# ACEfanatic02/par_raytracer

Hardware: AMD Instinct MI355X
Metric: Mrays/s at 1920x1080x8spp, 1M-tri OBJ (higher is better)
Workload: dtype f32; 1 GPU; C4: synthetic 1,002,528-triangle terrain OBJ (1,024 groups), 1920x1080, 8 spp, bounce_depth 2; seed=1234, triangles=1002528, width=1920, height=1080, spp=8, bounce_depth=2, rays_per_frame=77049910, parallelism=pixel rows sharded in 8-row blocks over 1 GPU(s), pipeline=pool, frames_in_flight=1

## Files before the change

par_raytracer_amd/csrc/dev_trace4.h:

```cpp
#pragma once

#include "dev_trace_common.h"

namespace prt {

struct TravRay {
    f3 o, d;
    float ix, iy, iz;
    float pnx, pny, pnz;
    HitRec best;
    int node, sp, kind;
};


enum { TRAV_SENTINEL = (int)0x80000000, TRAV_FLAG_NEAR = 1, TRAV_FLAG_OVERFLOW = 2, TRAV_SENTINEL_LAST = (int)0x80000003 };
PRT_D bool trav_done(int node) { return node <= TRAV_SENTINEL_LAST; }
PRT_D bool trav_flagged(int node) { return node <= TRAV_SENTINEL_LAST && node != TRAV_SENTINEL; }

typedef int StackEntry;
enum { STACK_ENTRY_INTS = 1, BVH_NODE_BYTES = 64, STACK_LDS_CAP_DEFAULT = 24 };

template <int BLOCK>
struct LdsStack {
    int * col;
    unsigned int cap;
    PRT_D void attach(int * lds, unsigned int tid) { col = lds + tid; }
    PRT_D int * frame_col() const { return col; }
    PRT_D bool push(int sp, int v) const {
        if ((unsigned int)sp < cap) { col[sp * BLOCK] = v; return true; }
        return false;
    }
    PRT_D int pop(int sp) const { return col[sp * BLOCK]; }
    PRT_D void flag(int bit) const { col[0] |= bit; }
};

template <int BLOCK>
struct LdsSpillStack {
    int * col;
    unsigned int cap;
    PRT_D void attach(int * lds, unsigned int tid) { col = lds + tid; }
    PRT_D int * frame_col() const { return col; }
    PRT_D void set_spill(int * base, unsigned int lanes) { spill = base; spill_stride = lanes; }
    int * spill;
    unsigned int spill_stride;
    PRT_D size_t spill_index(int sp) const {
        return (size_t)((unsigned int)sp - cap) * spill_stride + (blockIdx.x * (unsigned int)BLOCK + threadIdx.x);
    }
    PRT_D bool push(int sp, int v) const {
        if ((unsigned int)sp < cap) col[sp * BLOCK] = v;
        else spill[spill_index(sp)] = v;
        return true;
    }
    PRT_D int pop(int sp) const {
        if ((unsigned int)sp < cap) return col[sp * BLOCK];
        return spill[spill_index(sp)];
    }
    PRT_D void flag(int bit) const { col[0] |= bit; }
};

struct GlobalStack {
    int * col;
    size_t stride;
    PRT_D void attach(int * base, size_t lane, size_t lanes) { col = base + lane; stride = lanes; }
    PRT_D bool push(int sp, int v) const { col[(size_t)sp * stride] = v; return true; }
    PRT_D int pop(int sp) const { return col[(size_t)sp * stride]; }
    PRT_D void flag(int bit) const { col[0] |= bit; }
};

PRT_D void trav_idle(TravRay & r) { r.node = TRAV_SENTINEL; r.sp = 0; r.kind = 0; }
PRT_D bool trav_walking(const TravRay & r) { return r.node >= 0; }
PRT_D bool trav_done(const TravRay & r) { return trav_done(r.node); }

template <class STK> PRT_D int trav_end_flags(const TravRay & r, const STK &) { return trav_done(r.node) ? (r.node & 3) : 0; }
template <class STK> PRT_D bool trav_wants_resolve(const TravRay & r, const STK & stk) { return r.kind == TRACE_CLOSEST && (trav_end_flags(r, stk) & TRAV_FLAG_NEAR) != 0 && r.best.tri >= 0; }
template <class STK> PRT_D bool trav_needs_slow_path(const TravRay & r, const STK & stk) { return (trav_end_flags(r, stk) & TRAV_FLAG_OVERFLOW) != 0 || trav_wants_resolve(r, stk); }

template <class STK>
PRT_D void trav_pop(TravRay & r, const STK & stk) {
    r.sp--;
    r.node = stk.pop(r.sp);
}
template <class STK>
PRT_D void trav_push(TravRay & r, const STK & stk, int link) {
    if (stk.push(r.sp, link)) r.sp++;
    else stk.flag(TRAV_FLAG_OVERFLOW);
}

template <class STK>
PRT_D void trav_init(TravRay & r, f3 o, f3 d, int kind, float pad, const STK & stk) {
    r.o = o;
    r.d = d;
    const float tiny = 1e-30f;
    float dx = fabsf(d.x) < tiny ? (d.x < 0.0f ? -tiny : tiny) : d.x;
    float dy = fabsf(d.y) < tiny ? (d.y < 0.0f ? -tiny : tiny) : d.y;
    float dz = fabsf(d.z) < tiny ? (d.z < 0.0f ? -tiny : tiny) : d.z;
    r.ix = 1.0f / dx; r.iy = 1.0f / dy; r.iz = 1.0f / dz;
    r.pnx = (dx < 0.0f ? o.x - pad : o.x + pad) * r.ix;
    r.pny = (dy < 0.0f ? o.y - pad : o.y + pad) * r.iy;
    r.pnz = (dz < 0.0f ? o.z - pad : o.z + pad) * r.iz;
    r.best.t = 3.402823466e+38f;
    r.best.v = r.best.w = 0.0f;
    r.best.tri = -1;
    r.kind = kind;
    stk.push(0, TRAV_SENTINEL);
    r.sp = 1;
    r.node = 0;
}

PRT_D void cswap(float & ka, float & kb, int & la, int & lb) {
    const bool sw = kb < ka;
    const float k0 = sw ? kb : ka, k1 = sw ? ka : kb;
    const int l0 = sw ? lb : la, l1 = sw ? la : lb;
    ka = k0; kb = k1; la = l0; lb = l1;
}

template <class STK, bool COUNT>
PRT_D void trav_node_step(const DevScene & sc, TravRay & r, const STK & stk, TraceStats & st, float pad) {
    const uint4 * np = reinterpret_cast<const uint4 *>(reinterpret_cast<const char *>(sc.nodes) + ((unsigned int)r.node << 6));
    const uint4 w0 = np[0], w1 = np[1], w2 = np[2], w3 = np[3];
    if (COUNT) { st.nodes++; if (first_active_lane()) st.wnodes++; if ((unsigned int)r.sp > st.max_sp) st.max_sp = (unsigned int)r.sp; }
    const float kx = __uint_as_float(w0.w) * r.ix;
    const float ky = __uint_as_float(w3.z) * r.iy;
    const float kz = __uint_as_float(w3.w) * r.iz;
    const float ox = __uint_as_float(w0.x), oy = __uint_as_float(w0.y), oz = __uint_as_float(w0.z);
    const float pad2 = pad + pad;
    const float cnx = __builtin_fmaf(ox, r.ix, -r.pnx), cfx = __builtin_fmaf(pad2, fabsf(r.ix), cnx);
    const float cny = __builtin_fmaf(oy, r.iy, -r.pny), cfy = __builtin_fmaf(pad2, fabsf(r.iy), cny);
    const float cnz = __builtin_fmaf(oz, r.iz, -r.pnz), cfz = __builtin_fmaf(pad2, fabsf(r.iz), cnz);
    const bool sx = r.ix < 0.0f, sy = r.iy < 0.0f, sz = r.iz < 0.0f;
    const unsigned int qnx = sx ? w1.w : w1.x, qfx = sx ? w1.x : w1.w;
    const unsigned int qny = sy ? w2.x : w1.y, qfy = sy ? w1.y : w2.x;
    const unsigned int qnz = sz ? w2.y : w1.z, qfz = sz ? w1.z : w2.y;
    float key[4];
    int link[4] = { (int)w2.z, (int)w2.w, (int)w3.x, (int)w3.y };
    const float inf = __uint_as_float(0x7F800000u);
#pragma unroll
    for (int k = 0; k < 4; ++k) {
        const float nx = __builtin_fmaf((float)((qnx >> (8 * k)) & 0xFFu), kx, cnx);
        const float fx = __builtin_fmaf((float)((qfx >> (8 * k)) & 0xFFu), kx, cfx);
        const float ny = __builtin_fmaf((float)((qny >> (8 * k)) & 0xFFu), ky, cny);
        const float fy = __builtin_fmaf((float)((qfy >> (8 * k)) & 0xFFu), ky, cfy);
        const float nz = __builtin_fmaf((float)((qnz >> (8 * k)) & 0xFFu), kz, cnz);
        const float fz = __builtin_fmaf((float)((qfz >> (8 * k)) & 0xFFu), kz, cfz);
        const float tmin = fmaxf(fmaxf(fmaxf(nx, ny), nz), 0.0f);
        const float tmax = fminf(fminf(fminf(fx, fy), fz), r.best.t);
        key[k] = tmin <= tmax ? tmin : inf;
    }
    cswap(key[0], key[1], link[0], link[1]);
    cswap(key[2], key[3], link[2], link[3]);
    cswap(key[0], key[2], link[0], link[2]);
    cswap(key[1], key[3], link[1], link[3]);
    cswap(key[1], key[2], link[1], link[2]);
    if (key[0] < inf) {
        if (COUNT && first_active_lane()) st.wdescend++;
        if (COUNT) {
            const unsigned long long p3 = __ballot(key[3] < inf), p2 = __ballot(key[2] < inf), p1 = __ballot(key[1] < inf);
            if (first_active_lane()) st.wpush += (unsigned int)(p3 != 0ull) + (unsigned int)(p2 != 0ull) + (unsigned int)(p1 != 0ull);
        }
        if (key[3] < inf) trav_push(r, stk, link[3]);
        if (key[2] < inf) trav_push(r, stk, link[2]);
        if (key[1] < inf) trav_push(r, stk, link[1]);
        r.node = link[0];
    } else {
        if (COUNT && r.best.tri >= 0) st.culled++;
        if (COUNT && first_active_lane()) st.wpop++;
        trav_pop(r, stk);
    }
}

template <class STK, bool COUNT>
PRT_D bool trav_leaf(const DevScene & sc, TravRay & r, const STK & stk, TraceStats & st) {
    const f3 qp = r.o - (r.o + r.d);
    const unsigned int leaf = (unsigned int)~r.node;
    const unsigned int first = leaf >> 2, count = (leaf & 3u) + 1u;
    if (COUNT) { if (first_active_lane()) st.wleaves++; }
    int next_node = stk.pop(r.sp - 1);
    bool flagged = false;
    for (unsigned int i = 0; i < count; ++i) {
        const unsigned int ti = first + i;
        const float4 * tp = reinterpret_cast<const float4 *>(reinterpret_cast<const char *>(sc.tris) + ti * 48u);
        const float4 r0 = tp[0], r1 = tp[1], r2 = tp[2];
#if defined(__HIP_DEVICE_COMPILE__)
        asm volatile("" :: "v"(r0.x), "v"(r0.y), "v"(r0.z));
#endif
        if (COUNT) { st.tris++; if (first_active_lane()) st.wtris++; }
        float t, v, w;
        bool near;
        const bool hit = tri_test(r.o, r.d, qp, mk3(r0.x, r0.y, r0.z), mk3(r0.w, r1.x, r1.y), mk3(r1.z, r1.w, r2.x),
                                  mk3(r2.y, r2.z, r2.w), r.best.t, t, v, w, near);
        if (near) {
            stk.flag(TRAV_FLAG_NEAR);
            flagged = true;
        }
        if (hit) {
            r.best.t = t;
            r.best.v = v;
            r.best.w = w;
            r.best.tri = (int)ti;
            if (r.kind & TRACE_ANY) return true;
        }
    }
    if (flagged && r.sp == 1) next_node |= TRAV_FLAG_NEAR;
    r.sp--;
    r.node = next_node;
    return false;
}

template <class STK, bool COUNT>
PRT_D HitRec resolve_near_ties(const DevScene & sc, f3 o, f3 d, float pad, float min_t, const STK & stk, TraceStats & st) {
    TravRay r;
    HitRec result;
    result.t = 3.402823466e+38f; result.v = result.w = 0.0f; result.tri = -1;
    const f3 qp = o - (o + d);
    float bound = min_t * PRT_TIE_NEAR;
    for (unsigned int widen = 0; ; ++widen) {
        const bool last = widen >= sc.tie_widen_max;
        const float moat = bound * 1.00000095367431640625f;
        bool occupied = false;
        float best = 3.402823466e+38f;
        result.tri = -1;
        unsigned int next_rank = 0;
        RefSphereWalk walk;
        walk.reset();
        for (;;) {
            unsigned int c_rank = 0xFFFFFFFFu;
            int c_tri = -1;
            trav_init(r, o, d, TRACE_CLOSEST, pad, stk);
            r.best.t = moat;
            for (;;) {
                while (r.node >= 0) trav_node_step<STK, COUNT>(sc, r, stk, st, pad);
                if (trav_done(r.node)) break;
                const unsigned int leaf = (unsigned int)~r.node;
                const unsigned int first = leaf >> 2, count = (leaf & 3u) + 1u;
                for (unsigned int i = 0; i < count; ++i) {
                    const unsigned int ti = first + i;
                    const float4 * tp = sc.tris + 3 * (size_t)ti;
                    const float4 r0 = tp[0], r1 = tp[1], r2 = tp[2];
                    float t, dd, v, w;
                    if (!tri_geom(o, qp, mk3(r0.x, r0.y, r0.z), mk3(r0.w, r1.x, r1.y), mk3(r1.z, r1.w, r2.x), mk3(r2.y, r2.z, r2.w), t, dd, v, w)) continue;
                    const float th = t * (1.0f / dd);
                    if (th > bound) { if (th <= moat) occupied = true; continue; }
                    const unsigned int rk = sc.tri_rank[ti];
                    if (rk >= next_rank && rk < c_rank) { c_rank = rk; c_tri = (int)ti; }
                }
                trav_pop(r, stk);
            }
            if (c_tri < 0 || (occupied && !last)) break;
            const float4 * tp = sc.tris + 3 * (size_t)c_tri;
            const float4 r0 = tp[0], r1 = tp[1], r2 = tp[2];
            float t, v, w;
            if (walk.offers(sc, o, d, c_rank, best) &&
                tri_test_ref(o, qp, mk3(r0.x, r0.y, r0.z), mk3(r0.w, r1.x, r1.y), mk3(r1.z, r1.w, r2.x), mk3(r2.y, r2.z, r2.w), best, t, v, w)) {
                best = t;
                result.t = t; result.v = v; result.w = w; result.tri = c_tri;
            }
            next_rank = c_rank + 1u;
        }
        if (!occupied) break;
        if (last) {
            if (sc.near_tie_unresolved) atomicAdd(sc.near_tie_unresolved, 1ull);
            break;
        }
        bound = moat * PRT_TIE_NEAR;
    }
    return result;
}

template <class STK, bool COUNT>
PRT_D HitRec trace_ray(const DevScene & sc, f3 o, f3 d, int kind, float pad, const STK & stk, TraceStats & st) {
    TravRay r;
    trav_init(r, o, d, kind, pad, stk);
    for (;;) {
        while (r.node >= 0) trav_node_step<STK, COUNT>(sc, r, stk, st, pad);
        if (trav_done(r.node)) break;
        if (trav_leaf<STK, COUNT>(sc, r, stk, st)) return r.best;
    }
    if (kind == TRACE_CLOSEST && (r.node & TRAV_FLAG_NEAR) && r.best.tri >= 0) return resolve_near_ties<STK, COUNT>(sc, o, d, pad, r.best.t, stk, st);
    return r.best;
}

}
```

par_raytracer_amd/csrc/dev_trace8.h:

```cpp
#pragma once

#include "dev_trace_common.h"

namespace prt {

typedef int2 StackEntry;
enum { STACK_ENTRY_INTS = 2, BVH_NODE_BYTES = 80, STACK_LDS_CAP_DEFAULT = 13 };

struct TravRay {
    f3 o, d;
    float ix, iy, iz;
    float pnx, pny, pnz;
    HitRec best;
    int node;
    unsigned int tbase;
    unsigned int tbits;
    int sp, kind;
};

enum { TRAV_SENTINEL = (int)0x80000000, TRAV_FLAG_NEAR = 1, TRAV_FLAG_OVERFLOW = 2, TRAV_SENTINEL_LAST = (int)0x80000003 };

template <int BLOCK>
struct LdsStack {
    int * col;
    unsigned int cap;
    PRT_D void attach(int * lds, unsigned int tid) { col = lds + tid; }
    PRT_D int * frame_col() const { return col; }
    PRT_D bool put(int sp, int2 v) const {
        if ((unsigned int)sp < cap) { col[(2 * sp) * BLOCK] = v.x; col[(2 * sp + 1) * BLOCK] = v.y; return true; }
        return false;
    }
    PRT_D int2 get(int sp) const { return make_int2(col[(2 * sp) * BLOCK], col[(2 * sp + 1) * BLOCK]); }
    PRT_D void flag(int bit) const { col[0] |= bit; }
    PRT_D int marker() const { return col[0]; }
};

template <int BLOCK>
struct LdsSpillStack {
    int * col;
    unsigned int cap;
    int2 * spill;
    unsigned int spill_stride;
    PRT_D void attach(int * lds, unsigned int tid) { col = lds + tid; }
    PRT_D int * frame_col() const { return col; }
    PRT_D void set_spill(int * base, unsigned int lanes) { spill = reinterpret_cast<int2 *>(base); spill_stride = lanes; }
    PRT_D size_t spill_index(int sp) const {
        return (size_t)((unsigned int)sp - cap) * spill_stride + (blockIdx.x * (unsigned int)BLOCK + threadIdx.x);
    }
    PRT_D bool put(int sp, int2 v) const {
        if ((unsigned int)sp < cap) { col[(2 * sp) * BLOCK] = v.x; col[(2 * sp + 1) * BLOCK] = v.y; }
        else spill[spill_index(sp)] = v;
        return true;
    }
    PRT_D int2 get(int sp) const {
        if ((unsigned int)sp < cap) return make_int2(col[(2 * sp) * BLOCK], col[(2 * sp + 1) * BLOCK]);
        return spill[spill_index(sp)];
    }
    PRT_D void flag(int bit) const { col[0] |= bit; }
    PRT_D int marker() const { return col[0]; }
};

struct GlobalStack {
    int2 * col;
    size_t stride;
    PRT_D void attach(int * base, size_t lane, size_t lanes) { col = reinterpret_cast<int2 *>(base) + lane; stride = lanes; }
    PRT_D bool put(int sp, int2 v) const { col[(size_t)sp * stride] = v; return true; }
    PRT_D int2 get(int sp) const { return col[(size_t)sp * stride]; }
    PRT_D void flag(int bit) const { col[0].x |= bit; }
    PRT_D int marker() const { return col[0].x; }
};

PRT_D void trav_idle(TravRay & r) { r.node = TRAV_SENTINEL; r.tbits = 0u; r.tbase = 0u; r.sp = 0; r.kind = 0; }
PRT_D bool trav_at_leaf(const TravRay & r) { return (r.tbits & 0xFFu) != 0u; }
PRT_D bool trav_walking(const TravRay & r) { return (r.tbits & 0xFFu) == 0u && r.node >= 0; }
PRT_D bool trav_done(const TravRay & r) { return (r.tbits & 0xFFu) == 0u && r.node < 0; }

template <class STK> PRT_D int trav_end_flags(const TravRay & r, const STK & stk) {
    return ((r.kind & TRACE_ANY) && r.best.tri >= 0) ? 0 : (stk.marker() & 3);
}
template <class STK> PRT_D bool trav_wants_resolve(const TravRay & r, const STK & stk) {
    return !(r.kind & TRACE_ANY) && r.best.tri >= 0 && (stk.marker() & TRAV_FLAG_NEAR) != 0;
}
template <class STK> PRT_D bool trav_needs_slow_path(const TravRay & r, const STK & stk) {
    const int f = trav_end_flags(r, stk);
    return (f & TRAV_FLAG_OVERFLOW) != 0 || (!(r.kind & TRACE_ANY) && r.best.tri >= 0 && (f & TRAV_FLAG_NEAR) != 0);
}

template <class STK>
PRT_D void trav_init(TravRay & r, f3 o, f3 d, int kind, float pad, const STK & stk) {
    r.o = o;
    r.d = d;
    const float tiny = 1e-30f;
    float dx = fabsf(d.x) < tiny ? (d.x < 0.0f ? -tiny : tiny) : d.x;
    float dy = fabsf(d.y) < tiny ? (d.y < 0.0f ? -tiny : tiny) : d.y;
    float dz = fabsf(d.z) < tiny ? (d.z < 0.0f ? -tiny : tiny) : d.z;
    r.ix = 1.0f / dx; r.iy = 1.0f / dy; r.iz = 1.0f / dz;
    r.pnx = (dx < 0.0f ? o.x - pad : o.x + pad) * r.ix;
    r.pny = (dy < 0.0f ? o.y - pad : o.y + pad) * r.iy;
    r.pnz = (dz < 0.0f ? o.z - pad : o.z + pad) * r.iz;
    r.best.t = 3.402823466e+38f;
    r.best.v = r.best.w = 0.0f;
    r.best.tri = -1;
    const int oct = (dx < 0.0f ? 1 : 0) | (dy < 0.0f ? 2 : 0) | (dz < 0.0f ? 4 : 0);
    r.kind = kind | oct << 4;
    stk.put(0, make_int2(TRAV_SENTINEL, 0));
    r.sp = 1;
    r.node = 0;
    r.tbase = 0u;
    r.tbits = 0u;
}

template <class STK, bool COUNT>
PRT_D void trav_node_step(const DevScene & sc, TravRay & r, const STK & stk, TraceStats & st, float pad) {
    const uint4 * np = reinterpret_cast<const uint4 *>(reinterpret_cast<const char *>(sc.nodes) + (unsigned int)r.node * (unsigned int)BVH_NODE_BYTES);
    const uint4 q0 = np[0], q1 = np[1], q2 = np[2], q3 = np[3], q4 = np[4];
    if (COUNT) { st.nodes++; if (first_active_lane()) st.wnodes++; if ((unsigned int)r.sp > st.max_sp) st.max_sp = (unsigned int)r.sp; }
    const float kx = __uint_as_float(q0.w & 0x7F800000u) * r.ix;
    const float ky = __uint_as_float(q1.z & 0x7F800000u) * r.iy;
    const float kz = __uint_as_float(q1.w & 0x7F800000u) * r.iz;
    const float pad2 = pad + pad;
    const float cnx = __builtin_fmaf(__uint_as_float(q0.x), r.ix, -r.pnx), cfx = __builtin_fmaf(pad2, fabsf(r.ix), cnx);
    const float cny = __builtin_fmaf(__uint_as_float(q0.y), r.iy, -r.pny), cfy = __builtin_fmaf(pad2, fabsf(r.iy), cny);
    const float cnz = __builtin_fmaf(__uint_as_float(q0.z), r.iz, -r.pnz), cfz = __builtin_fmaf(pad2, fabsf(r.iz), cnz);
    const bool sx = r.ix < 0.0f, sy = r.iy < 0.0f, sz = r.iz < 0.0f;
    const unsigned int qnx[2] = { sx ? q3.z : q2.x, sx ? q3.w : q2.y }, qfx[2] = { sx ? q2.x : q3.z, sx ? q2.y : q3.w };
    const unsigned int qny[2] = { sy ? q4.x : q2.z, sy ? q4.y : q2.w }, qfy[2] = { sy ? q2.z : q4.x, sy ? q2.w : q4.y };
    const unsigned int qnz[2] = { sz ? q4.z : q3.x, sz ? q4.w : q3.y }, qfz[2] = { sz ? q3.x : q4.z, sz ? q3.y : q4.w };
    unsigned int m = 0u;
#pragma unroll
    for (int j = 7; j >= 0; --j) {
        const int h = j >> 2, k = j & 3;
        const float nx = __builtin_fmaf((float)((qnx[h] >> (8 * k)) & 0xFFu), kx, cnx);
        const float fx = __builtin_fmaf((float)((qfx[h] >> (8 * k)) & 0xFFu), kx, cfx);
        const float ny = __builtin_fmaf((float)((qny[h] >> (8 * k)) & 0xFFu), ky, cny);
        const float fy = __builtin_fmaf((float)((qfy[h] >> (8 * k)) & 0xFFu), ky, cfy);
        const float nz = __builtin_fmaf((float)((qnz[h] >> (8 * k)) & 0xFFu), kz, cnz);
        const float fz = __builtin_fmaf((float)((qfz[h] >> (8 * k)) & 0xFFu), kz, cfz);
        const float tmin = fmaxf(fmaxf(fmaxf(nx, ny), nz), 0.0f);
        const float tmax = fminf(fminf(fminf(fx, fy), fz), r.best.t);
#if defined(__HIP_DEVICE_COMPILE__)
        asm("v_cmp_le_f32 vcc, %1, %2\n\tv_addc_co_u32 %0, vcc, %0, %0, vcc" : "+v"(m) : "v"(tmin), "v"(tmax) : "vcc");
#else
        m = (m << 1) | (tmin <= tmax ? 1u : 0u);
#endif
    }
    const unsigned int imask = q0.w & 0xFFu;
    r.tbase = q1.y;
    r.tbits = (m & ~imask) | (q0.w & 0xFF00u) | (q1.z << 16);
    const unsigned int mi = m & imask;
    unsigned int gbase = q1.x, gbits = imask | mi << 8 | (q1.w & 3u) << 16;
    int at = r.sp;
    if (COUNT) {
        const unsigned long long down = __ballot(mi != 0u), all = __ballot(true);
        if (first_active_lane()) { st.wdescend += down != 0ull; st.wpop += down != all; }
    }
    if (mi == 0u) {
        if (COUNT && r.best.tri >= 0 && (m & ~imask) == 0u) st.culled++;
        at = r.sp - 1;
        const int2 e = stk.get(at);
        if (e.x <= TRAV_SENTINEL_LAST) {
            r.node = TRAV_SENTINEL;
            r.sp = at;
            return;
        }
        gbase = (unsigned int)e.x;
        gbits = (unsigned int)e.y;
    }
    const unsigned int rest8 = (gbits >> 8) & 0xFFu;
    const bool backwards = (((unsigned int)r.kind >> 4) >> ((gbits >> 16) & 3u)) & 1u;
    const unsigned int s = backwards ? 31u - (unsigned int)__clz((int)rest8) : (unsigned int)(__ffs((int)rest8) - 1);
    r.node = (int)(gbase + (unsigned int)__popc(gbits & ((1u << s) - 1u) & 0xFFu));
    gbits &= ~(0x100u << s);
    if (COUNT) {
        const unsigned long long pushing = __ballot(((gbits >> 8) & 0xFFu) != 0u);
        if (first_active_lane()) st.wpush += pushing != 0ull;
    }
    if ((gbits >> 8) & 0xFFu) {
        if (stk.put(at, make_int2((int)gbase, (int)gbits))) r.sp = at + 1;
        else { stk.flag(TRAV_FLAG_OVERFLOW); r.sp = at; }
    } else {
        r.sp = at;
    }
}

PRT_D void trav_leaf_range(const TravRay & r, unsigned int & first, unsigned int & count) {
    const unsigned int s = (unsigned int)(__ffs((int)(r.tbits & 0xFFu)) - 1);
    const unsigned int below = (1u << s) - 1u;
    const unsigned int ones = (unsigned int)__popc(r.tbits & (below << 8 | below << 16));
    const unsigned int twos = (unsigned int)__popc(r.tbits & (below << 24));
    first = r.tbase + ones + 2u * twos;
    count = 1u + ((r.tbits >> (16u + s)) & 1u) + 2u * ((r.tbits >> (24u + s)) & 1u);
}
PRT_D void trav_leaf_consume(TravRay & r) { r.tbits &= r.tbits - 1u; }

template <class STK, bool COUNT>
PRT_D bool trav_leaf(const DevScene & sc, TravRay & r, const STK & stk, TraceStats & st) {
    const f3 qp = r.o - (r.o + r.d);
    unsigned int first, count;
    trav_leaf_range(r, first, count);
    if (COUNT) { if (first_active_lane()) st.wleaves++; }
    for (unsigned int i = 0; i < count; ++i) {
        const unsigned int ti = first + i;
        const float4 * tp = reinterpret_cast<const float4 *>(reinterpret_cast<const char *>(sc.tris) + ti * 48u);
        const float4 r0 = tp[0], r1 = tp[1], r2 = tp[2];
#if defined(__HIP_DEVICE_COMPILE__)
        asm volatile("" :: "v"(r0.x), "v"(r0.y), "v"(r0.z));
#endif
        if (COUNT) { st.tris++; if (first_active_lane()) st.wtris++; }
        float t, v, w;
        bool near;
        const bool hit = tri_test(r.o, r.d, qp, mk3(r0.x, r0.y, r0.z), mk3(r0.w, r1.x, r1.y), mk3(r1.z, r1.w, r2.x),
                                  mk3(r2.y, r2.z, r2.w), r.best.t, t, v, w, near);
        if (near) stk.flag(TRAV_FLAG_NEAR);
        if (hit) {
            r.best.t = t;
            r.best.v = v;
            r.best.w = w;
            r.best.tri = (int)ti;
            if (r.kind & TRACE_ANY) return true;
        }
    }
    trav_leaf_consume(r);
    return false;
}

template <class STK, bool COUNT>
PRT_D HitRec resolve_near_ties(const DevScene & sc, f3 o, f3 d, float pad, float min_t, const STK & stk, TraceStats & st) {
    TravRay r;
    HitRec result;
    result.t = 3.402823466e+38f; result.v = result.w = 0.0f; result.tri = -1;
    const f3 qp = o - (o + d);
    float bound = min_t * PRT_TIE_NEAR;
    for (unsigned int widen = 0; ; ++widen) {
        const bool last = widen >= sc.tie_widen_max;
        const float moat = bound * 1.00000095367431640625f;
        bool occupied = false;
        float best = 3.402823466e+38f;
        result.tri = -1;
        unsigned int next_rank = 0;
        RefSphereWalk walk;
        walk.reset();
        for (;;) {
            unsigned int c_rank = 0xFFFFFFFFu;
            int c_tri = -1;
            trav_init(r, o, d, TRACE_CLOSEST, pad, stk);
            r.best.t = moat;
            for (;;) {
                while (trav_walking(r)) trav_node_step<STK, COUNT>(sc, r, stk, st, pad);
                if (trav_done(r)) break;
                unsigned int first, count;
                trav_leaf_range(r, first, count);
                for (unsigned int i = 0; i < count; ++i) {
                    const unsigned int ti = first + i;
                    const float4 * tp = sc.tris + 3 * (size_t)ti;
                    const float4 r0 = tp[0], r1 = tp[1], r2 = tp[2];
                    float t, dd, v, w;
                    if (!tri_geom(o, qp, mk3(r0.x, r0.y, r0.z), mk3(r0.w, r1.x, r1.y), mk3(r1.z, r1.w, r2.x), mk3(r2.y, r2.z, r2.w), t, dd, v, w)) continue;
                    const float th = t * (1.0f / dd);
                    if (th > bound) { if (th <= moat) occupied = true; continue; }
                    const unsigned int rk = sc.tri_rank[ti];
                    if (rk >= next_rank && rk < c_rank) { c_rank = rk; c_tri = (int)ti; }
                }
                trav_leaf_consume(r);
            }
            if (c_tri < 0 || (occupied && !last)) break;
            const float4 * tp = sc.tris + 3 * (size_t)c_tri;
            const float4 r0 = tp[0], r1 = tp[1], r2 = tp[2];
            float t, v, w;
            if (walk.offers(sc, o, d, c_rank, best) &&
                tri_test_ref(o, qp, mk3(r0.x, r0.y, r0.z), mk3(r0.w, r1.x, r1.y), mk3(r1.z, r1.w, r2.x), mk3(r2.y, r2.z, r2.w), best, t, v, w)) {
                best = t;
                result.t = t; result.v = v; result.w = w; result.tri = c_tri;
            }
            next_rank = c_rank + 1u;
        }
        if (!occupied) break;
        if (last) {
            if (sc.near_tie_unresolved) atomicAdd(sc.near_tie_unresolved, 1ull);
            break;
        }
        bound = moat * PRT_TIE_NEAR;
    }
    return result;
}

template <class STK, bool COUNT>
PRT_D HitRec trace_ray(const DevScene & sc, f3 o, f3 d, int kind, float pad, const STK & stk, TraceStats & st) {
    TravRay r;
    trav_init(r, o, d, kind, pad, stk);
    for (;;) {
        while (trav_walking(r)) trav_node_step<STK, COUNT>(sc, r, stk, st, pad);
        if (trav_done(r)) break;
        if (trav_leaf<STK, COUNT>(sc, r, stk, st)) return r.best;
    }
    if (trav_wants_resolve(r, stk)) return resolve_near_ties<STK, COUNT>(sc, o, d, pad, r.best.t, stk, st);
    return r.best;
}

}
```

par_raytracer_amd/csrc/kernels_pool.h:

```cpp
#pragma once

#include "kernels_wave.h"

namespace prt {

struct PoolBuffers {
    float4 * cq;
    float4 * hits;
    float4 * sq;
    unsigned int * head;
    unsigned int cap, scap;
    unsigned int topup_min;
    unsigned int topup_max;
    float4 * park;
    float4 * spark;
    unsigned int * park_count;
    unsigned int park_cap, spark_cap;
    unsigned int adopt;
    unsigned int * fin;
    float4 * scratch;
    float4 * jobsum;
    float4 * final_rgb;
    unsigned long long * wave_times;
    unsigned int guided, guided_min;
// ... 90 lines not shown
#endif
    return p;
}

PRT_D PoolArgs pool_args(const PoolArgs * args) {
    asm volatile("" : "+s"(args));
    PoolArgs A;
    __builtin_memcpy(&A, (PoolArgsPtr)args, sizeof(PoolArgs));
    A.sc.nodes = as_global(A.sc.nodes); A.sc.tris = as_global(A.sc.tris); A.sc.shade = as_global(A.sc.shade);
    A.sc.tri_rank = as_global(A.sc.tri_rank); A.sc.materials = as_global(A.sc.materials); A.sc.lights = as_global(A.sc.lights);
    A.sc.diffuse_dirs = as_global(A.sc.diffuse_dirs); A.sc.spec_dirs = as_global(A.sc.spec_dirs);
    A.sc.textures = as_global(A.sc.textures); A.sc.texels = as_global(A.sc.texels); A.sc.srgb_lut = as_global(A.sc.srgb_lut);
    A.sc.tri_uv = as_global(A.sc.tri_uv); A.sc.tri_tan = as_global(A.sc.tri_tan);
    A.P.pixel_list = as_global(A.P.pixel_list); A.P.stack_spill = as_global(A.P.stack_spill);
    A.B.accum = as_global(A.B.accum); A.B.rng = as_global(A.B.rng); A.B.rng_aux = as_global(A.B.rng_aux); A.B.ring = as_global(A.B.ring);
    A.B.frames = as_global(A.B.frames);
    A.Q.cq = as_global(A.Q.cq); A.Q.hits = as_global(A.Q.hits); A.Q.sq = as_global(A.Q.sq); A.Q.head = as_global(A.Q.head);
    A.Q.park = as_global(A.Q.park); A.Q.spark = as_global(A.Q.spark); A.Q.park_count = as_global(A.Q.park_count);
    A.Q.fin = as_global(A.Q.fin); A.Q.scratch = as_global(A.Q.scratch); A.Q.jobsum = as_global(A.Q.jobsum); A.Q.final_rgb = as_global(A.Q.final_rgb);
    A.Q.wave_times = as_global(A.Q.wave_times);
    return A;
}

template <int BLOCK, bool EXACT> struct PoolStack { typedef LdsStack<BLOCK> type; };
template <int BLOCK> struct PoolStack<BLOCK, true> { typedef LdsSpillStack<BLOCK> type; };
template <int BLOCK> PRT_D void pool_stack_spill(LdsStack<BLOCK> &, PoolArgsPtr) {}
template <int BLOCK> PRT_D void pool_stack_spill(LdsSpillStack<BLOCK> & stack, PoolArgsPtr args) {
    stack.set_spill(as_global(args->P.stack_spill), args->P.stack_spill_stride);
}

__global__ void k_pool_store_args(PoolArgs a, PoolArgs * dst, unsigned int * zero, unsigned int n_zero, unsigned int * adopt_head,
                                  unsigned int adopt_cap_div) {
    if (threadIdx.x < n_zero) zero[threadIdx.x] = 0u;
    if (threadIdx.x == 0 && blockIdx.x == 0) {
        dst[0] = a;
        if (adopt_head) {
            a.Q.adopt = 1;
            a.Q.head = adopt_head;
            a.Q.cap /= adopt_cap_div;
            a.Q.scap /= adopt_cap_div;
            dst[1] = a;
        }
    }
}

template <int BLOCK, int WAVES, bool LDSTAB, bool RING, bool COUNT, bool TEX, bool ADAPT, int RINGMEM, bool EXACT, bool SHARED>
__global__ __launch_bounds__(BLOCK, WAVES) void k_pool(const PoolArgs * args, DevCounters * ctr) {
    static_assert(!(SHARED && EXACT), "the adopting EXACT launch keeps wave-private pools");
    extern __shared__ int s_stack[];
    constexpr int LDS_MATS = 32, LDS_LIGHTS = 4;
    __shared__ float4 s_diffuse[LDSTAB ? 1024 : 1];
    __shared__ DevMaterial s_mats[LDS_MATS];
    __shared__ DevLight s_lights[LDS_LIGHTS];
    __shared__ unsigned long long s_red[2];
    __shared__ unsigned int s_ctl[SHARED ? PCTL_WORDS : 1];
    __shared__ unsigned int s_rg[COUNT ? 2 * PRT_REGION_COUNT : 1];
    {
        const PoolArgs A0 = pool_args(args);
        const DevScene & sc = A0.sc;
        if (LDSTAB) for (unsigned int k = threadIdx.x; k < 1024u; k += BLOCK) s_diffuse[k] = sc.diffuse_dirs[k];
        if (sc.material_count <= (unsigned int)LDS_MATS) {
            const float4 * src = reinterpret_cast<const float4 *>(sc.materials);
            float4 * dst = reinterpret_cast<float4 *>(s_mats);
            for (unsigned int k = threadIdx.x; k < sc.material_count * 4u; k += BLOCK) dst[k] = src[k];
        }
        if (sc.light_count <= (unsigned int)LDS_LIGHTS) {
            const float4 * src = reinterpret_cast<const float4 *>(sc.lights);
            float4 * dst = reinterpret_cast<float4 *>(s_lights);
            for (unsigned int k = threadIdx.x; k < sc.light_count * 3u; k += BLOCK) dst[k] = src[k];
        }
    }
    if (threadIdx.x < 2) s_red[threadIdx.x] = 0ull;
    if (SHARED && threadIdx.x < (unsigned int)PCTL_WORDS) s_ctl[threadIdx.x] = 0u;
    if (COUNT) for (unsigned int k = threadIdx.x; k < 2u * PRT_REGION_COUNT; k += BLOCK) s_rg[k] = 0u;
    const RegionTable rg = (RegionTable)s_rg;
    __syncthreads();

    const unsigned int slot_id = blockIdx.x * BLOCK + threadIdx.x;
    const unsigned int lane = lane_id();
    const unsigned int wave = SHARED ? blockIdx.x : (unsigned int)__builtin_amdgcn_readfirstlane((int)(slot_id >> 6));
    constexpr unsigned int ULANES = SHARED ? (unsigned int)BLOCK : 64u;
    const unsigned int ulane = SHARED ? threadIdx.x : lane;
    const bool lead_wave = !SHARED || (unsigned int)__builtin_amdgcn_readfirstlane((int)(threadIdx.x >> 6)) == 0u;
    typedef typename PoolStack<BLOCK, EXACT>::type Stack;
    Stack stack;
    stack.attach(s_stack, threadIdx.x);
    stack.cap = ((PoolArgsPtr)args)->P.stack_lds_entries;
    pool_stack_spill(stack, (PoolArgsPtr)args);

    unsigned int n_f = 0;
    unsigned int n_spec = 0;
    int cur = 0;
    unsigned int n_c = 0, n_s = 0;
    bool fetch_done = false;
    unsigned long long rays = 0ull;
    unsigned int shaded_w = 0;
    unsigned int elided_w = 0;
    TraceStats st;
    st.nodes = st.tris = st.wnodes = st.wleaves = st.wtris = st.wrefills = st.wrays = st.max_sp = st.culled = 0;

#define PRT_POOL_LISTS(A)                                                                              \
    const unsigned int cap = (A).Q.cap, scap = (A).Q.scap;                                            \
    float4 * const cq_base = (A).Q.cq + (size_t)wave * 6u * cap;                                      \
    float4 * const hits = (A).Q.hits + (size_t)wave * cap;                                            \
    float4 * const sq_o = (A).Q.sq + (size_t)wave * 3u * scap;                                        \
    float4 * const sq_c = sq_o + scap;                                                                \
    float4 * const sq_d = sq_c + scap;                                                                \
    float4 * const co = cq_base + (size_t)cur * 3u * cap;                                             \
    float4 * const cd = co + cap;                                                                     \
    float4 * const ct = cd + cap;                                                                     \
    (void)hits; (void)sq_o; (void)sq_c; (void)sq_d; (void)ct

    unsigned long long ph_topup = 0ull, ph_trace = 0ull, ph_shade = 0ull, ph_final = 0ull;
    unsigned long long dry_steps = 0ull, dry_rays = 0ull;
    const unsigned long long ph_begin = COUNT ? __builtin_readcyclecounter() : 0ull;
    const unsigned long long wt_begin = COUNT ? wall_clock64() : 0ull;
    unsigned long long wt_dry = 0ull;
    region_count<COUNT>(rg, PRT_REGION_WAVE);
    for (;;) {
        const unsigned long long ph_t0 = COUNT ? __builtin_readcyclecounter() : 0ull;
        region_count<COUNT>(rg, PRT_REGION_ROUND);
        if (!fetch_done) {
          const PoolArgs A = pool_args(args);
          const DevParams & P = A.P;
          const WaveBuffers & B = A.B;
          const PoolBuffers & Q = A.Q;
          PRT_POOL_LISTS(A);
          if (EXACT && Q.adopt) {
            if (n_c + n_s + n_f == 0u) {
                const unsigned int n_parked = *Q.park_count < Q.park_cap ? *Q.park_count : Q.park_cap;
                const unsigned int n_waves = gridDim.x * (BLOCK / 64);
                unsigned int chunk = (n_parked + n_waves - 1u) / n_waves;
                chunk = chunk < 1u ? 1u : chunk > cap ? cap : chunk;
                unsigned int base = 0;
                if (lane == 0) base = atomicAdd(Q.head, chunk);
                base = (unsigned int)__builtin_amdgcn_readfirstlane((int)base);
                if (base >= n_parked) {
                    fetch_done = true;
                } else {
                    unsigned int cnt = n_parked - base;
                    if (cnt <= chunk) fetch_done = true; else cnt = chunk;
                    unsigned int * const fin_list = ADAPT ? Q.fin + (size_t)wave * cap : nullptr;
                    unsigned int m_c = 0, m_f = 0;
                    for (unsigned int k0 = 0; k0 < cnt; k0 += 64u) {
                        const unsigned int k = k0 + lane;
                        const bool have = k < cnt;
                        float4 e0 = make_float4(0, 0, 0, 0), e1 = e0, e2 = e0;
                        if (have) { e0 = Q.park[base + k]; e1 = Q.park[(size_t)Q.park_cap + base + k]; e2 = Q.park[2u * (size_t)Q.park_cap + base + k]; }
                        const bool is_fin = ADAPT && have && as_i(e2.w) == POOL_PARK_FINALISE;
                        const bool is_ray = have && !is_fin;
                        const unsigned long long mr = __ballot(is_ray), mf = __ballot(is_fin);
                        const unsigned int pr = __builtin_amdgcn_mbcnt_hi((unsigned int)(mr >> 32), __builtin_amdgcn_mbcnt_lo((unsigned int)mr, 0u));
                        const unsigned int pf = __builtin_amdgcn_mbcnt_hi((unsigned int)(mf >> 32), __builtin_amdgcn_mbcnt_lo((unsigned int)mf, 0u));
                        if (is_ray) { co[m_c + pr] = e0; cd[m_c + pr] = e1; ct[m_c + pr] = make_float4(e2.x, e2.y, e2.z, 0.0f); }
                        if (is_fin) {
                            const unsigned int j = (unsigned int)as_i(e0.w);
                            fin_list[m_f + pf] = j;
                            float4 js = Q.jobsum[j];
                            js.w = as_f(as_i(js.w) & 0x7FFFFFFF);
                            Q.jobsum[j] = js;
                        }
                        m_c += (unsigned int)__popcll(mr);
                        m_f += (unsigned int)__popcll(mf);
                    }
                    cnt = m_c;
                    n_f = m_f;
                    n_c = cnt;
                    rays -= cnt;
                }
            }
          } else if (n_c + n_f - n_spec + (!SHARED && Q.guided ? (Q.guided_min < Q.topup_min ? Q.guided_min : Q.topup_min) : Q.topup_min) <= cap) {
            const unsigned int room = cap - (n_c + n_f - n_spec);
            unsigned int want = room < Q.topup_max ? room : Q.topup_max;
            if (!SHARED && Q.guided) {
                const unsigned int taken = __hip_atomic_load(Q.head, __ATOMIC_RELAXED, __HIP_MEMORY_SCOPE_AGENT);
                const unsigned int left = taken < B.n_samples ? B.n_samples - taken : 0u;
                const unsigned int n_units = gridDim.x * (unsigned int)(BLOCK / 64);
                unsigned int lim = (unsigned int)(((unsigned long long)left * Q.guided) / (8ull * n_units));
                if (lim < Q.guided_min) lim = Q.guided_min;
                if (room < (lim < Q.topup_min ? lim : Q.topup_min)) want = 0u;
                else if (want > lim) want = lim;
            }
            if (want != 0u) {
            unsigned int base = 0;
            if (SHARED) {
                if (threadIdx.x == 0) s_ctl[PCTL_TOPUP_BASE] = atomicAdd(Q.head, want);
                __syncthreads();
                base = s_ctl[PCTL_TOPUP_BASE];
                __syncthreads();
            } else if (lane == 0) base = atomicAdd(Q.head, want);
            base = (unsigned int)__builtin_amdgcn_readfirstlane((int)base);
            if (base >= B.n_samples) {
                fetch_done = true;
            } else {
                unsigned int cnt = B.n_samples - base;
                if (cnt <= want) fetch_done = true; else cnt = want;
                const DevCamera cam = A.cam;
                region_count<COUNT>(rg, PRT_REGION_TOPUP);
                for (unsigned int k = ulane; k < cnt; k += ULANES) {
                    region_count<COUNT>(rg, PRT_REGION_TOPUP_PASS);
                    const unsigned int sid = base + k;
                    const unsigned int gsid = B.sample_base + sid;
                    SampleState S;
                    Frame fr;
                    u64 * ring = RING && RINGMEM != 0 ? B.ring + (size_t)sid * B.ring_step : nullptr;
                    if (ADAPT) {
                        sample_begin<RING>(cam, P, pixel_of_local(P, gsid), 0u, S, fr, ring, B.ring_stride);
                        Q.jobsum[sid] = make_float4(0.0f, 0.0f, 0.0f, as_f(0));
                    } else {
                        sample_begin<RING>(cam, P, pixel_of_local(P, gsid / P.spp), gsid % P.spp, S, fr, ring, B.ring_stride);
                    }
                    B.rng[sid] = make_ulonglong2(S.rng.chain, S.rng.prev);
                    if (RING && RINGMEM != 0) B.rng_aux[sid] = make_ulonglong2(S.rng.seed0, (u64)S.rng.k);
                    co[n_c + k] = make_float4(fr.ray_o.x, fr.ray_o.y, fr.ray_o.z, as_f((int)sid));
                    cd[n_c + k] = make_float4(fr.ray_d.x, fr.ray_d.y, fr.ray_d.z, as_f((int)WF_PENDING_FRESH_BIT << 8));
                    ct[n_c + k] = make_float4(1.0f, 1.0f, 1.0f, 0.0f);
                }
                n_c += cnt;
            }
            }
          }
        }
        if (COUNT && fetch_done && wt_dry == 0ull) wt_dry = wall_clock64();
        const unsigned int total = n_c + n_s;
        if (total == 0u && n_f == 0u) {
            if (fetch_done) break;
            continue;
        }
        pool_sync<SHARED>();
        if (lead_wave) rays += total;
        const unsigned long long ph_t1 = COUNT ? __builtin_readcyclecounter() : 0ull;

        {
            const PoolArgs A = pool_args(args);
            const DevScene & sc = A.sc;
            const DevParams & P = A.P;
            const WaveBuffers & B = A.B;
            const int keep_min = A.keep_min, node_min = A.node_min, node_frac = A.node_frac;
            PRT_POOL_LISTS(A);
            const DevLight * lights = sc.light_count <= (unsigned int)LDS_LIGHTS ? s_lights : sc.lights;
            TravRay r;
            trav_idle(r);
            int ray = -1;
            float4 payload = make_float4(0, 0, 0, 0);
            int sample = 0;
            unsigned int next = 0;
            bool dry = total == 0u;
            for (;;) {
                region_count<COUNT>(rg, PRT_REGION_TRACE_OUTER);
                const unsigned long long idle = __ballot(ray < 0);
                if (idle != 0ull && !dry) {
                    if (COUNT && lane == 0) st.wrefills++;
                    const unsigned int prefix = __builtin_amdgcn_mbcnt_hi((unsigned int)(idle >> 32), __builtin_amdgcn_mbcnt_lo((unsigned int)idle, 0u));
                    const unsigned int n_idle = (unsigned int)__popcll(idle);
                    if (SHARED) {
                        unsigned int b = 0;
                        if (lane == 0) b = atomicAdd(&s_ctl[PCTL_TRACE_NEXT], n_idle);
                        next = (unsigned int)__builtin_amdgcn_readfirstlane((int)b);
                        if (next > total) next = total;
                    }
                    const unsigned int avail = total - next;
                    const unsigned int take = n_idle < avail ? n_idle : avail;
                    if (ray < 0 && prefix < take) {
                        region_count<COUNT>(rg, PRT_REGION_REFILL);
                        const unsigned int idx = next + prefix;
                        float4 ro, rd;
                        int kind;
                        if (idx < n_c) {
                            ro = co[idx];
                            rd = cd[idx];
                            kind = WF_KIND_CLOSEST;
                        } else {
                            const unsigned int j = idx - n_c;
                            ro = sq_o[j];
                            payload = sq_c[j];
                            if (payload.w < 0.0f) {
                                const DevLight & L = lights[(unsigned int)(-payload.w) - 1u];
                                const f3 lv = mk3(L.facing[0], L.facing[1], L.facing[2]) * -1.0f;
                                rd = make_float4(lv.x, lv.y, lv.z, 0.0f);
                                kind = WF_KIND_SHADOW_ANY;
                            } else {
                                rd = sq_d[j];
                                kind = WF_KIND_SHADOW_DIST;
                            }
                        }
                        sample = as_i(ro.w);
                        const f3 d = mk3(rd.x, rd.y, rd.z);
                        const f3 ob = mk3(ro.x, ro.y, ro.z) + d * P.ray_bias;
                        trav_init(r, ob, d, kind == WF_KIND_SHADOW_ANY ? TRACE_ANY : TRACE_CLOSEST, P.box_pad, stack);
                        ray = (int)idx;
                    }
                    next += take;
                    dry = next == total;
                }
                const int leave_below = dry ? 1 : keep_min;
                if (__ballot(ray >= 0) == 0ull) break;

                while (ray >= 0) {
                    region_count<COUNT>(rg, PRT_REGION_WALK_PASS);
                    const int walkers = __popcll(__ballot(trav_walking(r)));
                    const int wfrac = (walkers * node_frac) >> 3;
                    const int nmin = node_min < wfrac ? node_min : wfrac;
                    const unsigned int with_ray = COUNT ? (unsigned int)__popcll(__ballot(true)) : 0u;
                    while (trav_walking(r)) {
                        trav_node_step<Stack, COUNT>(sc, r, stack, st, P.box_pad);
                        if (COUNT && first_active_lane()) { st.wrays += with_ray; if (dry) { dry_steps += 1ull; dry_rays += with_ray; } }
                        if (__popcll(__ballot(trav_walking(r))) < nmin) break;
                    }
                    bool fin = trav_done(r);
                    if (!fin && !trav_walking(r)) fin = trav_leaf<Stack, COUNT>(sc, r, stack, st);
                    if (fin) {
                        region_count<COUNT>(rg, PRT_REGION_FINISH);
                        if (EXACT && trav_wants_resolve(r, stack)) r.best = resolve_near_ties<Stack, COUNT>(sc, r.o, r.d, P.box_pad, r.best.t, stack, st);
                        if (!EXACT && trav_needs_slow_path(r, stack)) {
                            region_count<COUNT>(rg, PRT_REGION_PARK);
                            if (ADAPT && (unsigned int)ray < n_c && ((unsigned int)as_i(cd[ray].w) >> 8 & POOL_SPEC_PENDING_BIT)) {
                                hits[ray] = make_float4(0.0f, 0.0f, 0.0f, as_f(POOL_CANCELLED_MARK));
                            } else if ((unsigned int)ray < n_c) {
                                const unsigned int slot = atomicAdd(A.Q.park_count, 1u);
                                if (slot < A.Q.park_cap) {
                                    const float4 t4 = ct[ray];
                                    A.Q.park[slot] = co[ray];
                                    A.Q.park[(size_t)A.Q.park_cap + slot] = cd[ray];
                                    A.Q.park[2u * (size_t)A.Q.park_cap + slot] = make_float4(t4.x, t4.y, t4.z, as_f(POOL_PARK_CLOSEST));
                                }
                                hits[ray] = make_float4(0.0f, 0.0f, 0.0f, as_f(POOL_PARKED_MARK));
                            } else {
                                const unsigned int slot = atomicAdd(A.Q.park_count + 1, 1u);
                                if (slot < A.Q.spark_cap) {
                                    A.Q.spark[slot] = sq_o[(unsigned int)ray - n_c];
                                    A.Q.spark[(size_t)A.Q.spark_cap + slot] = payload;
                                    A.Q.spark[2u * (size_t)A.Q.spark_cap + slot] = make_float4(r.d.x, r.d.y, r.d.z, 0.0f);
                                }
                                if (ADAPT) {
                                    float * const w = &A.Q.jobsum[sample].w;
                                    *w = as_f(as_i(*w) | (int)0x80000000);
                                }
                            }
                        } else if ((unsigned int)ray < n_c) {
                            hits[ray] = make_float4(r.best.t, r.best.v, r.best.w, as_f(r.best.tri));
                        } else {
                            const bool lit = r.best.tri < 0 || (payload.w >= 0.0f && r.best.t * r.best.t <= payload.w);
                            if (lit) {
                                accum_add(B.accum + sample, mk3(payload.x, payload.y, payload.z));
                            }
                        }
                        ray = -1;
                        break;
                    }
                    if (__popcll(__ballot(true)) < leave_below) break;
                }
            }
        }
        pool_sync<SHARED>();
        const unsigned long long ph_t2 = COUNT ? __builtin_readcyclecounter() : 0ull;

        {
            const PoolArgs A = pool_args(args);
            const DevScene & sc = A.sc;
            const DevParams & P = A.P;
            const WaveBuffers & B = A.B;
            const PoolBuffers & Q = A.Q;
            PRT_POOL_LISTS(A);
            unsigned int * const fin = ADAPT ? Q.fin + (size_t)wave * cap : nullptr;
            ShadeTables tb;
            tb.diffuse = LDSTAB ? s_diffuse : sc.diffuse_dirs;
            tb.materials = sc.material_count <= (unsigned int)LDS_MATS ? s_mats : sc.materials;
            tb.lights = sc.light_count <= (unsigned int)LDS_LIGHTS ? s_lights : sc.lights;
            const int nxt = cur ^ 1;
            PoolEmit<ADAPT, SHARED, COUNT> emit;
            emit.rg = rg;
            emit.co = cq_base + (size_t)nxt * 3u * cap;
            emit.cd = emit.co + cap;
            emit.ct = emit.cd + cap;
            emit.so = sq_o; emit.sc = sq_c; emit.sd = sq_d;
            emit.fin = fin;
            emit.m_c = 0; emit.m_s = 0; emit.m_f = 0; emit.m_elided = 0;
            emit.s_cnt = SHARED ? &s_ctl[PCTL_CNT + 4 * nxt] : nullptr;
            if (SHARED && threadIdx.x < 4u) {
                s_ctl[PCTL_CNT + 4 * cur + threadIdx.x] = 0u;
                if (threadIdx.x == 0) s_ctl[PCTL_TRACE_NEXT] = 0u;
            }
            const unsigned int b_first = SHARED ? (threadIdx.x >> 6) * 64u : 0u;
            if (ADAPT) {
                float4 * const scratch = Q.scratch;
#define POOL_SCRATCH_AT(k, j) ((size_t)(j) * P.max_spp + (k))
                const unsigned long long ph_f0 = COUNT ? __builtin_readcyclecounter() : 0ull;
                for (unsigned int b0 = b_first; b0 < n_f; b0 += ULANES) {
                    const unsigned int i = b0 + lane;
                    const bool live = i < n_f;
                    bool go_on = false;
                    unsigned int j = 0;
                    f3 ray_o = mk3(0, 0, 0), ray_d = mk3(0, 0, 1);
                    if (live) {
                        j = fin[i];
                    }
                    int job = 0;
                    unsigned int spec_idx = 0;
                    float4 spec_off = make_float4(0.0f, 0.0f, 0.0f, 0.0f);
                    if (live) {
                        job = as_i(Q.jobsum[j].w);
                        if (job & (POOL_JOB_SPEC_FLYING | POOL_JOB_SPEC_DRAWN)) {
                            spec_off = Q.final_rgb[j];
                            spec_idx = (unsigned int)as_i(spec_off.z);
                            if ((job & POOL_JOB_SPEC_FLYING) && as_i(hits[spec_idx].w) == POOL_CANCELLED_MARK)
                                job = (job & ~POOL_JOB_SPEC_FLYING) | POOL_JOB_SPEC_DRAWN;
                        }
                    }
                    bool defer = false;
                    if (live && !EXACT) {
                        defer = (job & POOL_JOB_DEFERRED) != 0;
                        if (defer) {
                            const unsigned int slot = atomicAdd(Q.park_count, 1u);
                            if (slot < Q.park_cap) {
                                Q.park[slot] = make_float4(0.0f, 0.0f, 0.0f, as_f((int)j));
                                Q.park[(size_t)Q.park_cap + slot] = make_float4(0.0f, 0.0f, 0.0f, 0.0f);
                                Q.park[2u * (size_t)Q.park_cap + slot] = make_float4(0.0f, 0.0f, 0.0f, as_f(POOL_PARK_FINALISE));
                            }
                            if (job & POOL_JOB_SPEC_FLYING) {
                                hits[spec_idx].w = as_f(POOL_CANCELLED_MARK);
                                job = (job & ~POOL_JOB_SPEC_FLYING) | POOL_JOB_SPEC_DRAWN;
                            }
                            Q.jobsum[j].w = as_f(job);
                        }
                    }
                    if (live && !defer) {
                        const f3 a = accum_read(B.accum + j);
                        const float4 st = Q.jobsum[j];
                        unsigned int samp = (unsigned int)(job & POOL_JOB_SAMPLE_MASK);
                        const f3 sum_prev = mk3(st.x, st.y, st.z);
                        const f3 c = a;
                        const float sq_prev = samp ? scratch[POOL_SCRATCH_AT(samp - 1u, j)].w : 0.0f;
                        scratch[POOL_SCRATCH_AT(samp, j)] = make_float4(c.x, c.y, c.z, sq_prev + ((c.x * c.x + c.y * c.y) + c.z * c.z));
                        const f3 sum = sum_prev + c;
                        bool stop = false;
                        bool decided = false;
                        if (samp >= P.spp) {
                            const float n = (float)samp;
                            const float bound = sq_prev - ((sum_prev.x * sum_prev.x + sum_prev.y * sum_prev.y) + sum_prev.z * sum_prev.z) / n;
                            decided = bound - 2e-5f * sq_prev > P.variance_threshold * (n - 1.0f) * 1.001f + 1e-30f;
                        }
                        if (samp >= P.spp && !decided) {
                            const f3 mean = sum_prev / (float)samp;
                            float variance = 0.0f;
                            unsigned int k = 0;
                            for (; k + 8u <= samp; k += 8u) {
                                float4 v[8];
#pragma unroll
                                for (int u = 0; u < 8; ++u) v[u] = scratch[POOL_SCRATCH_AT(k + (unsigned int)u, j)];
#pragma unroll
                                for (int u = 0; u < 8; ++u) {
                                    const float d = (fabsf(v[u].x - mean.x) + fabsf(v[u].y - mean.y)) + fabsf(v[u].z - mean.z);
                                    variance += d * d;
                                }
                            }
                            for (; k < samp; ++k) {
                                const float4 v = scratch[POOL_SCRATCH_AT(k, j)];
                                const float d = (fabsf(v.x - mean.x) + fabsf(v.y - mean.y)) + fabsf(v.z - mean.z);
                                variance += d * d;
                            }
                            variance /= (float)(samp - 1u);
                            stop = variance <= P.variance_threshold;
                            if (fabsf(variance - P.variance_threshold) <= 1e-3f * P.variance_threshold + 1e-7f) atomicAdd(&ctr->variance_close_calls, 1ull);
                        }
                        if (!stop) {
                            ++samp;
                            stop = samp >= P.max_spp;
                        }
                        if (stop) {
                            if (job & POOL_JOB_SPEC_FLYING) hits[spec_idx].w = as_f(POOL_CANCELLED_MARK);
                            const f3 out = sum / (float)samp;
                            Q.final_rgb[j] = make_float4(out.x, out.y, out.z, 1.0f);
                        } else {
                            Q.jobsum[j] = make_float4(sum.x, sum.y, sum.z, as_f((int)samp));
                            if (!(job & POOL_JOB_SPEC_FLYING)) {
                                float off_x, off_y;
                                if (job & POOL_JOB_SPEC_DRAWN) {
// ... 202 lines not shown
```

Measured before the change: 6885 Mrays/s.

## Batch near-tie candidates per traversal and carry known hit distance through park

The near-tie resolver now collects up to four lowest-rank candidate triangles per BVH traversal instead of one, so fewer full re-traversals are needed to walk the rank order. Parked closest-hit rays also store their already-found hit distance, and when they are replayed on the exact path the traversal is skipped and goes straight to tie resolution. This cuts repeated traversal work on the slow path, at the cost of more registers for the candidate arrays and extra state passed through the park queue.

```diff
diff --git a/par_raytracer_amd/csrc/dev_trace4.h b/par_raytracer_amd/csrc/dev_trace4.h
--- a/par_raytracer_amd/csrc/dev_trace4.h
+++ b/par_raytracer_amd/csrc/dev_trace4.h
@@ -105,6 +105,14 @@
     stk.push(0, TRAV_SENTINEL);
     r.sp = 1;
     r.node = 0;
+}
+
+template <class STK>
+PRT_D void trav_set_near_tied(TravRay & r, float t, const STK &) {
+    r.best.t = t;
+    r.best.tri = 0;
+    r.node = TRAV_SENTINEL | TRAV_FLAG_NEAR;
+    r.sp = 0;
 }
 
 PRT_D void cswap(float & ka, float & kb, int & la, int & lb) {
@@ -206,6 +214,7 @@
     return false;
 }
 
+enum { TIE_BATCH = 4 };
 template <class STK, bool COUNT>
 PRT_D HitRec resolve_near_ties(const DevScene & sc, f3 o, f3 d, float pad, float min_t, const STK & stk, TraceStats & st) {
     TravRay r;
@@ -223,8 +232,10 @@
         RefSphereWalk walk;
         walk.reset();
         for (;;) {
-            unsigned int c_rank = 0xFFFFFFFFu;
-            int c_tri = -1;
+            unsigned int c_rank[TIE_BATCH];
+            int c_tri[TIE_BATCH];
+#pragma unroll
+            for (int k = 0; k < TIE_BATCH; ++k) { c_rank[k] = 0xFFFFFFFFu; c_tri[k] = -1; }
             trav_init(r, o, d, TRACE_CLOSEST, pad, stk);
             r.best.t = moat;
             for (;;) {
@@ -241,20 +252,39 @@
                     const float th = t * (1.0f / dd);
                     if (th > bound) { if (th <= moat) occupied = true; continue; }
                     const unsigned int rk = sc.tri_rank[ti];
-                    if (rk >= next_rank && rk < c_rank) { c_rank = rk; c_tri = (int)ti; }
+                    bool fresh = rk >= next_rank && rk < c_rank[TIE_BATCH - 1];
+#pragma unroll
+                    for (int k = 0; k < TIE_BATCH - 1; ++k) fresh = fresh && rk != c_rank[k];
+                    if (fresh) {
+                        c_rank[TIE_BATCH - 1] = rk; c_tri[TIE_BATCH - 1] = (int)ti;
+#pragma unroll
+                        for (int k = TIE_BATCH - 1; k > 0; --k) {
+                            const bool sw = c_rank[k] < c_rank[k - 1];
+                            const unsigned int r0k = sw ? c_rank[k] : c_rank[k - 1], r1k = sw ? c_rank[k - 1] : c_rank[k];
+                            const int t0k = sw ? c_tri[k] : c_tri[k - 1], t1k = sw ? c_tri[k - 1] : c_tri[k];
+                            c_rank[k - 1] = r0k; c_rank[k] = r1k; c_tri[k - 1] = t0k; c_tri[k] = t1k;
+                        }
+                    }
                 }
                 trav_pop(r, stk);
             }
-            if (c_tri < 0 || (occupied && !last)) break;
-            const float4 * tp = sc.tris + 3 * (size_t)c_tri;
-            const float4 r0 = tp[0], r1 = tp[1], r2 = tp[2];
-            float t, v, w;
-            if (walk.offers(sc, o, d, c_rank, best) &&
-                tri_test_ref(o, qp, mk3(r0.x, r0.y, r0.z), mk3(r0.w, r1.x, r1.y), mk3(r1.z, r1.w, r2.x), mk3(r2.y, r2.z, r2.w), best, t, v, w)) {
-                best = t;
-                result.t = t; result.v = v; result.w = w; result.tri = c_tri;
+            if (c_tri[0] < 0 || (occupied && !last)) break;
+            const bool full = c_tri[TIE_BATCH - 1] >= 0;
+            while (c_tri[0] >= 0) {
+                const float4 * tp = sc.tris + 3 * (size_t)c_tri[0];
+                const float4 r0 = tp[0], r1 = tp[1], r2 = tp[2];
+                float t, v, w;
+                if (walk.offers(sc, o, d, c_rank[0], best) &&
+                    tri_test_ref(o, qp, mk3(r0.x, r0.y, r0.z), mk3(r0.w, r1.x, r1.y), mk3(r1.z, r1.w, r2.x), mk3(r2.y, r2.z, r2.w), best, t, v, w)) {
+                    best = t;
+                    result.t = t; result.v = v; result.w = w; result.tri = c_tri[0];
+                }
+                next_rank = c_rank[0] + 1u;
+#pragma unroll
+                for (int k = 0; k < TIE_BATCH - 1; ++k) { c_rank[k] = c_rank[k + 1]; c_tri[k] = c_tri[k + 1]; }
+                c_tri[TIE_BATCH - 1] = -1;
             }
-            next_rank = c_rank + 1u;
+            if (!full) break;
         }
         if (!occupied) break;
         if (last) {
diff --git a/par_raytracer_amd/csrc/dev_trace8.h b/par_raytracer_amd/csrc/dev_trace8.h
--- a/par_raytracer_amd/csrc/dev_trace8.h
+++ b/par_raytracer_amd/csrc/dev_trace8.h
@@ -108,6 +108,15 @@
     r.node = 0;
     r.tbase = 0u;
     r.tbits = 0u;
+}
+
+template <class STK>
+PRT_D void trav_set_near_tied(TravRay & r, float t, const STK & stk) {
+    r.best.t = t;
+    r.best.tri = 0;
+    r.node = TRAV_SENTINEL;
+    r.sp = 0;
+    stk.flag(TRAV_FLAG_NEAR);
 }
 
 template <class STK, bool COUNT>
@@ -224,6 +233,7 @@
     return false;
 }
 
+enum { TIE_BATCH = 4 };
 template <class STK, bool COUNT>
 PRT_D HitRec resolve_near_ties(const DevScene & sc, f3 o, f3 d, float pad, float min_t, const STK & stk, TraceStats & st) {
     TravRay r;
@@ -241,8 +251,10 @@
         RefSphereWalk walk;
         walk.reset();
         for (;;) {
-            unsigned int c_rank = 0xFFFFFFFFu;
-            int c_tri = -1;
+            unsigned int c_rank[TIE_BATCH];
+            int c_tri[TIE_BATCH];
+#pragma unroll
+            for (int k = 0; k < TIE_BATCH; ++k) { c_rank[k] = 0xFFFFFFFFu; c_tri[k] = -1; }
             trav_init(r, o, d, TRACE_CLOSEST, pad, stk);
             r.best.t = moat;
             for (;;) {
@@ -259,20 +271,39 @@
                     const float th = t * (1.0f / dd);
                     if (th > bound) { if (th <= moat) occupied = true; continue; }
                     const unsigned int rk = sc.tri_rank[ti];
-                    if (rk >= next_rank && rk < c_rank) { c_rank = rk; c_tri = (int)ti; }
+                    bool fresh = rk >= next_rank && rk < c_rank[TIE_BATCH - 1];
+#pragma unroll
+                    for (int k = 0; k < TIE_BATCH - 1; ++k) fresh = fresh && rk != c_rank[k];
+                    if (fresh) {
+                        c_rank[TIE_BATCH - 1] = rk; c_tri[TIE_BATCH - 1] = (int)ti;
+#pragma unroll
+                        for (int k = TIE_BATCH - 1; k > 0; --k) {
+                            const bool sw = c_rank[k] < c_rank[k - 1];
+                            const unsigned int r0k = sw ? c_rank[k] : c_rank[k - 1], r1k = sw ? c_rank[k - 1] : c_rank[k];
+                            const int t0k = sw ? c_tri[k] : c_tri[k - 1], t1k = sw ? c_tri[k - 1] : c_tri[k];
+                            c_rank[k - 1] = r0k; c_rank[k] = r1k; c_tri[k - 1] = t0k; c_tri[k] = t1k;
+                        }
+                    }
                 }
                 trav_leaf_consume(r);
             }
-            if (c_tri < 0 || (occupied && !last)) break;
-            const float4 * tp = sc.tris + 3 * (size_t)c_tri;
-            const float4 r0 = tp[0], r1 = tp[1], r2 = tp[2];
-            float t, v, w;
-            if (walk.offers(sc, o, d, c_rank, best) &&
-                tri_test_ref(o, qp, mk3(r0.x, r0.y, r0.z), mk3(r0.w, r1.x, r1.y), mk3(r1.z, r1.w, r2.x), mk3(r2.y, r2.z, r2.w), best, t, v, w)) {
-                best = t;
-                result.t = t; result.v = v; result.w = w; result.tri = c_tri;
+            if (c_tri[0] < 0 || (occupied && !last)) break;
+            const bool full = c_tri[TIE_BATCH - 1] >= 0;
+            while (c_tri[0] >= 0) {
+                const float4 * tp = sc.tris + 3 * (size_t)c_tri[0];
+                const float4 r0 = tp[0], r1 = tp[1], r2 = tp[2];
+                float t, v, w;
+                if (walk.offers(sc, o, d, c_rank[0], best) &&
+                    tri_test_ref(o, qp, mk3(r0.x, r0.y, r0.z), mk3(r0.w, r1.x, r1.y), mk3(r1.z, r1.w, r2.x), mk3(r2.y, r2.z, r2.w), best, t, v, w)) {
+                    best = t;
+                    result.t = t; result.v = v; result.w = w; result.tri = c_tri[0];
+                }
+                next_rank = c_rank[0] + 1u;
+#pragma unroll
+                for (int k = 0; k < TIE_BATCH - 1; ++k) { c_rank[k] = c_rank[k + 1]; c_tri[k] = c_tri[k + 1]; }
+                c_tri[TIE_BATCH - 1] = -1;
             }
-            next_rank = c_rank + 1u;
+            if (!full) break;
         }
         if (!occupied) break;
         if (last) {
diff --git a/par_raytracer_amd/csrc/kernels_pool.h b/par_raytracer_amd/csrc/kernels_pool.h
--- a/par_raytracer_amd/csrc/kernels_pool.h
+++ b/par_raytracer_amd/csrc/kernels_pool.h
@@ -266,7 +266,7 @@
                         const unsigned long long mr = __ballot(is_ray), mf = __ballot(is_fin);
                         const unsigned int pr = __builtin_amdgcn_mbcnt_hi((unsigned int)(mr >> 32), __builtin_amdgcn_mbcnt_lo((unsigned int)mr, 0u));
                         const unsigned int pf = __builtin_amdgcn_mbcnt_hi((unsigned int)(mf >> 32), __builtin_amdgcn_mbcnt_lo((unsigned int)mf, 0u));
-                        if (is_ray) { co[m_c + pr] = e0; cd[m_c + pr] = e1; ct[m_c + pr] = make_float4(e2.x, e2.y, e2.z, 0.0f); }
+                        if (is_ray) { co[m_c + pr] = e0; cd[m_c + pr] = e1; ct[m_c + pr] = e2; }
                         if (is_fin) {
                             const unsigned int j = (unsigned int)as_i(e0.w);
                             fin_list[m_f + pf] = j;
@@ -402,6 +402,10 @@
                         const f3 d = mk3(rd.x, rd.y, rd.z);
                         const f3 ob = mk3(ro.x, ro.y, ro.z) + d * P.ray_bias;
                         trav_init(r, ob, d, kind == WF_KIND_SHADOW_ANY ? TRACE_ANY : TRACE_CLOSEST, P.box_pad, stack);
+                        if (EXACT && kind == WF_KIND_CLOSEST) {
+                            const float t_known = ct[idx].w;
+                            if (t_known != 0.0f) trav_set_near_tied(r, t_known, stack);
+                        }
                         ray = (int)idx;
                     }
                     next += take;
@@ -436,7 +440,8 @@
                                     const float4 t4 = ct[ray];
                                     A.Q.park[slot] = co[ray];
                                     A.Q.park[(size_t)A.Q.park_cap + slot] = cd[ray];
-                                    A.Q.park[2u * (size_t)A.Q.park_cap + slot] = make_float4(t4.x, t4.y, t4.z, as_f(POOL_PARK_CLOSEST));
+                                    const bool t_known = !(trav_end_flags(r, stack) & TRAV_FLAG_OVERFLOW) && as_i(r.best.t) > POOL_PARK_FINALISE;
+                                    A.Q.park[2u * (size_t)A.Q.park_cap + slot] = make_float4(t4.x, t4.y, t4.z, t_known ? r.best.t : as_f(POOL_PARK_CLOSEST));
                                 }
                                 hits[ray] = make_float4(0.0f, 0.0f, 0.0f, as_f(POOL_PARKED_MARK));
                             } else {
```

Result: no change. 6918 Mrays/s, median of 6 (+0.5%).
